# hedgepigdaniel/video-annotator

Hardware: AMD Instinct MI355X
Metric: stabilized frames/sec at 4K NV12, 1/2/4/8 GPU; remap % HBM roofline (higher is better)
Workload: dtype u8 pixels / f32 map / f64 rotations

## Files before the change

video-annotator_amd/csrc/vstab_warp_fused.hip:

```cpp
#include <algorithm>
#include <climits>
#include <cmath>
#include <cstdlib>

#include <hip/hip_ext.h>

#include "vstab_device.hpp"
#include "vstab_device10.hpp"
#include "vstab_internal.hpp"
#include "vstab_warp_args.hpp"
#include "vstab_warp_tile.hpp"

namespace vstab {

#ifdef VSTAB_DEV
#define VSTAB_STAMP(k)                                                                                                   \
    if (ta.timing && lane == 0) ta.timing[((size_t)blockIdx.x * 4 + (size_t)wave) * 8 + (k)] = __builtin_amdgcn_s_memrealtime()
#else
#define VSTAB_STAMP(k)
#endif

template <int RWB, int RW, int MODE, int FMT, bool CACHED, bool SPLIT, int DEPTH = 8, int BLEND = 0>
__device__ __forceinline__ bool warp_tile(const FusedArgs &ta, uint32_t *smem, const int x0, const int y0) {
    static_assert((DEPTH == 8 && FMT < 2) || (DEPTH == 10 && FMT >= 2), "10-bit pixels leave as 16-bit BGR (FMT 2) or P010 planes (FMT 3)");
    using SrcVec = typename std::conditional<DEPTH == 10, uint4, uint2>::type;
    constexpr uint32_t BPS = DEPTH == 10 ? 2 : 1;
    constexpr int TH = 4 * RW;
    constexpr int STAGE_MAX = StageTrips<RWB, RW>::value;
    constexpr int QB = CACHED ? 0 : QMAGIC_BITS;
    constexpr bool PIX8 = DEPTH == 10 && BLEND == VSTAB_BLEND_FP16;
    constexpr int PD = PIX8 ? 2 : 1;
    constexpr bool RS = map_mode_is_rs(MODE);
    constexpr int BASE = map_mode_base(MODE);
    uint32_t *const tile = smem + 8;
    const WarpArgs &a = ta.w;
    const int tid = threadIdx.x, lane = tid & 63, wave = __builtin_amdgcn_readfirstlane(tid >> 6);
    const float rfx = rcp_refined(a.p.ofx), rfy = rcp_refined(a.p.ofy);

    VSTAB_STAMP(0);
    if (wave == 0) {
        __builtin_amdgcn_s_setprio(3);
        probe_tile<TH, STAGE_MAX, MODE, CACHED>(ta, x0, y0, lane, rfx, rfy, smem);
        __builtin_amdgcn_s_setprio(VSTAB_WARP_PRIO);
    }
    __syncthreads();
    const int bx0 = __builtin_amdgcn_readfirstlane((int)smem[0]), by0 = __builtin_amdgcn_readfirstlane((int)smem[1]);
    const int wb = __builtin_amdgcn_readfirstlane((int)smem[2]), hb = __builtin_amdgcn_readfirstlane((int)smem[3]);
    const int box_state = __builtin_amdgcn_readfirstlane((int)smem[4]);
    if constexpr (SPLIT) {
        if (box_state == 2) return false;
    }
    const bool use_lds = box_state == 1;
    const int x = x0 + lane;
    VSTAB_STAMP(1);

    const int ux_n = wb >> 3, units = use_lds ? ux_n * (hb >> 1) : 0;
#ifdef VSTAB_DEV
    const int pw = (wb + ta.lds_pad) * PD;
#else
    const int pw = wb * PD;
#endif
    SrcVec y0w[STAGE_MAX], y1w[STAGE_MAX], uvw[STAGE_MAX];
    int ldsoff[STAGE_MAX];
    constexpr int ZERO_BLOCK = 1 << 24;
    if (use_lds) {
        const float rn = __builtin_amdgcn_rcpf((float)ux_n);
        int uy = (int)((float)tid * rn), ux = tid - uy * ux_n;
        if (ux < 0) ux += ux_n, uy--;
        if (ux >= ux_n) ux -= ux_n, uy++;
        int sy_ = (int)(256.0f * rn), sx_ = 256 - sy_ * ux_n;
        if (sx_ < 0) sx_ += ux_n, sy_--;
        if (sx_ >= ux_n) sx_ -= ux_n, sy_++;
        const uint32_t pitch_y = (uint32_t)a.pitch_y, pitch_uv = (uint32_t)a.pitch_uv;
#pragma unroll
        for (int it = 0; it < STAGE_MAX; it++) {
            if (it > 0 && units <= it * 256) {
                y0w[it] = y1w[it] = uvw[it] = SrcVec(), ldsoff[it] = -1;
                continue;
            }
            const bool valid = tid + it * 256 < units;
            const int gx = bx0 + 8 * ux, gy = by0 + 2 * uy;
            const bool inside = (uint32_t)gx < (uint32_t)(a.sw & ~7) && (uint32_t)gy < (uint32_t)a.sh;
            const uint32_t cx = (uint32_t)min(max(gx, 0), (a.sw & ~7) - 8), cy = (uint32_t)min(max(gy, 0), a.sh - 2);
            const uint32_t oy = __umul24(cy, pitch_y) + cx * BPS, ouv = __umul24(cy >> 1, pitch_uv) + cx * BPS;
            y0w[it] = *reinterpret_cast<const SrcVec *>(a.y + oy);
            y1w[it] = *reinterpret_cast<const SrcVec *>(a.y + (oy + pitch_y));
            uvw[it] = *reinterpret_cast<const SrcVec *>(a.uv + ouv);
            ldsoff[it] = valid ? (__mul24(2 * uy, pw) + 8 * PD * ux) | (inside ? 0 : ZERO_BLOCK) : -1;
            ux += sx_, uy += sy_;
            if (ux >= ux_n) ux -= ux_n, uy++;
        }
    } else {
#pragma unroll
        for (int it = 0; it < STAGE_MAX; it++) y0w[it] = y1w[it] = uvw[it] = SrcVec(), ldsoff[it] = -1;
    }

    VSTAB_STAMP(2);
    int qxb[RW], qyb[RW];
    {
        int unused_cx[RW / 2], unused_cy[RW / 2];
        const float unused_qm[4] = {QMAGIC, QMAGIC, QMAGIC, QMAGIC};
        map_phase<RW, MODE, CACHED, false>(ta, x, y0, wave, lane, rfx, rfy, qxb, qyb, unused_cx, unused_cy, unused_qm);
    }
#pragma unroll
    for (int j = 0; j < RW; j++) asm volatile("" : "+v"(qxb[j]), "+v"(qyb[j]) : : "memory");

    VSTAB_STAMP(3);
    if (use_lds) {
#pragma unroll
        for (int it = 0; it < STAGE_MAX; it++) {
            if (ldsoff[it] >= ZERO_BLOCK) {
                uint32_t *d = tile + (ldsoff[it] - ZERO_BLOCK);
                const uint4 z = make_uint4(0, 0, 0, 0);
#pragma unroll
                for (int q = 0; q < 2 * PD; q++) *reinterpret_cast<uint4 *>(d + 4 * q) = z, *reinterpret_cast<uint4 *>(d + pw + 4 * q) = z;
#ifdef VSTAB_DEV
            } else if (DEPTH == 8 && ldsoff[it] >= 0 && (ta.ablate & 4)) {
                uint32_t *d = tile + ldsoff[it];
                *reinterpret_cast<uint4 *>(d) = make_uint4(y0w[it].x, y0w[it].y, uvw[it].x, uvw[it].y);
                *reinterpret_cast<uint4 *>(d + 4) = make_uint4(y0w[it].y, y0w[it].x, uvw[it].x, uvw[it].y);
                *reinterpret_cast<uint4 *>(d + pw) = make_uint4(y1w[it].x, y1w[it].y, uvw[it].x, uvw[it].y);
                *reinterpret_cast<uint4 *>(d + pw + 4) = make_uint4(y1w[it].y, y1w[it].x, uvw[it].y, uvw[it].x);
#endif
            } else if (ldsoff[it] >= 0) {
                uint32_t *d = tile + ldsoff[it];
                if constexpr (DEPTH == 10) {
                    const uint32_t ya[4] = {y0w[it].x, y0w[it].y, y0w[it].z, y0w[it].w}, yb[4] = {y1w[it].x, y1w[it].y, y1w[it].z, y1w[it].w};
                    const uint32_t cw[4] = {uvw[it].x, uvw[it].y, uvw[it].z, uvw[it].w};
#pragma unroll
                    for (int half = 0; half < 2; half++) {
                        const ChromaTerm c0 = chroma_term10(cw[2 * half]), c1 = chroma_term10(cw[2 * half + 1]);
                        if constexpr (PIX8) {
                            const uint32_t la = ya[2 * half], lb = ya[2 * half + 1], ma = yb[2 * half], mb = yb[2 * half + 1];
                            const uint2 a0 = pack_bgr10h((int)((la & 0xffffu) >> 6), c0), a1 = pack_bgr10h((int)(la >> 22), c0);
                            const uint2 a2 = pack_bgr10h((int)((lb & 0xffffu) >> 6), c1), a3 = pack_bgr10h((int)(lb >> 22), c1);
                            const uint2 b0 = pack_bgr10h((int)((ma & 0xffffu) >> 6), c0), b1 = pack_bgr10h((int)(ma >> 22), c0);
                            const uint2 b2 = pack_bgr10h((int)((mb & 0xffffu) >> 6), c1), b3 = pack_bgr10h((int)(mb >> 22), c1);
                            *reinterpret_cast<uint4 *>(d + 8 * half) = make_uint4(a0.x, a0.y, a1.x, a1.y);
                            *reinterpret_cast<uint4 *>(d + 8 * half + 4) = make_uint4(a2.x, a2.y, a3.x, a3.y);
                            *reinterpret_cast<uint4 *>(d + pw + 8 * half) = make_uint4(b0.x, b0.y, b1.x, b1.y);
                            *reinterpret_cast<uint4 *>(d + pw + 8 * half + 4) = make_uint4(b2.x, b2.y, b3.x, b3.y);
                            continue;
                        }
                        uint4 r0, r1;
                        r0.x = pack_bgr10((int)((ya[2 * half] & 0xffffu) >> 6), c0), r0.y = pack_bgr10((int)(ya[2 * half] >> 22), c0);
                        r0.z = pack_bgr10((int)((ya[2 * half + 1] & 0xffffu) >> 6), c1), r0.w = pack_bgr10((int)(ya[2 * half + 1] >> 22), c1);
                        r1.x = pack_bgr10((int)((yb[2 * half] & 0xffffu) >> 6), c0), r1.y = pack_bgr10((int)(yb[2 * half] >> 22), c0);
                        r1.z = pack_bgr10((int)((yb[2 * half + 1] & 0xffffu) >> 6), c1), r1.w = pack_bgr10((int)(yb[2 * half + 1] >> 22), c1);
                        *reinterpret_cast<uint4 *>(d + 4 * half) = r0;
                        *reinterpret_cast<uint4 *>(d + pw + 4 * half) = r1;
                    }
                } else
#pragma unroll
                for (int half = 0; half < 2; half++) {
                    const uint32_t cw = half ? uvw[it].y : uvw[it].x, ya = half ? y0w[it].y : y0w[it].x, yb = half ? y1w[it].y : y1w[it].x;
                    const ChromaTerm c0 = chroma_term_folded(cw & 255, (cw >> 8) & 255);
                    const ChromaTerm c1 = chroma_term_folded((cw >> 16) & 255, cw >> 24);
                    uint4 r0, r1;
                    r0.x = pack_bgrx(ya & 255, c0), r0.y = pack_bgrx((ya >> 8) & 255, c0);
                    r0.z = pack_bgrx((ya >> 16) & 255, c1), r0.w = pack_bgrx(ya >> 24, c1);
                    r1.x = pack_bgrx(yb & 255, c0), r1.y = pack_bgrx((yb >> 8) & 255, c0);
                    r1.z = pack_bgrx((yb >> 16) & 255, c1), r1.w = pack_bgrx(yb >> 24, c1);
                    *reinterpret_cast<uint4 *>(d + 4 * half) = r0;
                    *reinterpret_cast<uint4 *>(d + pw + 4 * half) = r1;
                }
            }
        }
    }
    VSTAB_STAMP(4);
    __syncthreads();
    VSTAB_STAMP(5);

    const bool col_live = x < a.dw;
    uint32_t out[RW];
    {
        int cx = bx0 + (QB >> 5), cy = by0 + (QB >> 5);
        asm("" : "+s"(cx), "+s"(cy));
        const uint32_t wlim = use_lds ? (uint32_t)(wb - 1) : 0u, hlim = (uint32_t)(hb - 1);
        int Xr[RW], Yr[RW];
        const uint32_t wb4 = (uint32_t)pw << 2;
        uint32_t tile_lds = (uint32_t)(uintptr_t)(__attribute__((address_space(3))) uint32_t *)tile;
        asm("" : "+s"(tile_lds));
        uint32_t mxx = 0, mxy = 0;
#pragma unroll
        for (int j = 0; j < RW; j++) {
            Xr[j] = (qxb[j] >> 5) - cx, Yr[j] = (qyb[j] >> 5) - cy;
            mxx = max(mxx, (uint32_t)Xr[j]), mxy = max(mxy, (uint32_t)Yr[j]);
        }
        if (!__builtin_amdgcn_ballot_w64(mxx >= wlim || mxy >= hlim)) {
            constexpr int TG = RW < TAP_GROUP ? RW : TAP_GROUP;
            if constexpr (PIX8) {
#pragma unroll
                for (int j0 = 0; j0 < RW; j0 += TG) {
                    uint2 t0[TG], t1[TG], t2[TG], t3[TG];
#pragma unroll
                    for (int j = 0; j < TG; j++) {
                        uint32_t ax8, au;
                        asm("v_lshl_add_u32 %0, %1, 3, %2" : "=v"(ax8) : "v"(Xr[j0 + j]), "s"(tile_lds));
                        asm("v_mad_u32_u24 %0, %1, %2, %3" : "=v"(au) : "v"(Yr[j0 + j]), "s"(wb4), "v"(ax8));
                        const LdsPair *u = reinterpret_cast<const LdsPair *>(au), *l = reinterpret_cast<const LdsPair *>(au + wb4);
                        const u32x2 v0 = u[0], v1 = u[1], v2 = l[0], v3 = l[1];
                        t0[j] = make_uint2(v0.x, v0.y), t1[j] = make_uint2(v1.x, v1.y), t2[j] = make_uint2(v2.x, v2.y), t3[j] = make_uint2(v3.x, v3.y);
                    }
#pragma unroll
                    for (int j = 0; j < TG; j++) out[j0 + j] = blend_bgr10h(t0[j], t1[j], t2[j], t3[j], qxb[j0 + j] & 31, qyb[j0 + j] & 31);
                }
            } else
#pragma unroll
            for (int j0 = 0; j0 < RW; j0 += TG) {
                uint32_t t0[TG], t1[TG], t2[TG], t3[TG];
#pragma unroll
                for (int j = 0; j < TG; j++) {
                    uint32_t ax4, au;
                    asm("v_lshl_add_u32 %0, %1, 2, %2" : "=v"(ax4) : "v"(Xr[j0 + j]), "s"(tile_lds));
                    asm("v_mad_u32_u24 %0, %1, %2, %3" : "=v"(au) : "v"(Yr[j0 + j]), "s"(wb4), "v"(ax4));
                    const LdsWord *u = reinterpret_cast<const LdsWord *>(au), *l = reinterpret_cast<const LdsWord *>(au + wb4);
                    t0[j] = u[0], t1[j] = u[1], t2[j] = l[0], t3[j] = l[1];
                }
#pragma unroll
                for (int j = 0; j < TG; j++) {
#ifdef VSTAB_DEV
                    if (ta.ablate & 2) out[j0 + j] = t0[j] ^ t1[j] ^ t2[j] ^ t3[j] ^ (qxb[j0 + j] & 31) ^ (qyb[j0 + j] & 31);
                    else
#endif
                    out[j0 + j] = DEPTH == 10 ? blend_bgr10<BLEND>(t0[j], t1[j], t2[j], t3[j], qxb[j0 + j] & 31, qyb[j0 + j] & 31)
                                              : blend_bgrx(t0[j], t1[j], t2[j], t3[j], qxb[j0 + j] & 31, qyb[j0 + j] & 31);
                }
            }
        } else {
            uint32_t slow = 0;
#pragma unroll
            for (int j = 0; j < RW; j++) {
                const bool inbox = (uint32_t)Xr[j] < wlim && (uint32_t)Yr[j] < hlim;
                uint32_t v = 0;
                if (inbox) {
                    const uint32_t *t = tile + (__mul24(Yr[j], pw) + PD * Xr[j]);
                    if constexpr (PIX8)
                        v = blend_bgr10h(make_uint2(t[0], t[1]), make_uint2(t[2], t[3]), make_uint2(t[pw], t[pw + 1]), make_uint2(t[pw + 2], t[pw + 3]), qxb[j] & 31,
                                         qyb[j] & 31);
                    else
                        v = DEPTH == 10 ? blend_bgr10<BLEND>(t[0], t[1], t[pw], t[pw + 1], qxb[j] & 31, qyb[j] & 31)
                                        : blend_bgrx(t[0], t[1], t[pw], t[pw + 1], qxb[j] & 31, qyb[j] & 31);
                }
                out[j] = v;
                const bool live = col_live && y0 + wave * RW + j < a.dh;
                slow |= (!inbox && live ? 1u : 0u) << j;
            }
            if (__builtin_amdgcn_ballot_w64(slow != 0)) {
#pragma unroll 1
                for (int j = 0; j < RW; j++) {
                    int sx = qxb[0], sy = qyb[0];
#pragma unroll
                    for (int k = 1; k < RW; k++) sx = j == k ? qxb[k] : sx, sy = j == k ? qyb[k] : sy;
                    if ((slow >> j) & 1u) {
                        const uint32_t v = DEPTH == 10 ? gather_pixel10<BLEND>(a, sx - QB, sy - QB) : gather_pixel_far(a, sx - QB, sy - QB);
#pragma unroll
                        for (int k = 0; k < RW; k++) out[k] = j == k ? v : out[k];
                    }
                }
            }
        }
    }

    VSTAB_STAMP(6);
#ifdef VSTAB_DEV
    if (ta.ablate & 8) {
        uint32_t acc = 0;
#pragma unroll
        for (int j = 0; j < RW; j++) acc ^= out[j];
        if (acc == 0x12345678u) a.dst[0] = 1;
        return true;
    }
#endif
    const int ncols = min(64, a.dw - x0);
    if constexpr (FMT == 2) {
#pragma unroll
        for (int j = 0; j < RW; j++) {
            const int y = y0 + wave * RW + j;
            if (y >= a.dh) break;
            if (col_live) {
                uint16_t *o = reinterpret_cast<uint16_t *>(a.dst + ((size_t)(uint32_t)y * a.pitch_dst + (uint32_t)x * 6u));
                o[0] = (uint16_t)(out[j] & 1023u), o[1] = (uint16_t)((out[j] >> 10) & 1023u), o[2] = (uint16_t)(out[j] >> 20);
            }
        }
    } else if constexpr (FMT == 3) {
#pragma unroll
        for (int j = 0; j < RW; j++) {
            const int y = y0 + wave * RW + j;
            if (y >= a.dh) break;
            const int B = (int)(out[j] & 1023u), G = (int)((out[j] >> 10) & 1023u), R = (int)(out[j] >> 20);
            const uint32_t yb = (uint32_t)sat10((CRY * R + CGY * G + CBY * B + (1 << 19) + (64 << 20)) >> 20) << 6;
            const uint32_t y1 = (uint32_t)__builtin_amdgcn_mov_dpp((int)yb, 0x55, 0xf, 0xf, true);
            const uint32_t y2 = (uint32_t)__builtin_amdgcn_mov_dpp((int)yb, 0xaa, 0xf, 0xf, true);
            const uint32_t y3 = (uint32_t)__builtin_amdgcn_mov_dpp((int)yb, 0xff, 0xf, 0xf, true);
            uint16_t *o = reinterpret_cast<uint16_t *>(a.dst + (size_t)(uint32_t)y * a.pitch_dst) + x;
            if (!(lane & 3) && col_live) {
                if (ta.dst_vec_ok && x + 4 <= a.dw) {
                    *reinterpret_cast<uint2 *>(o) = make_uint2(yb | (y1 << 16), y2 | (y3 << 16));
                } else {
                    const uint32_t w[4] = {yb, y1, y2, y3};
                    for (int i = 0; i < 4 && x + i < a.dw; i++) o[i] = (uint16_t)w[i];
                }
            }
            if (!(y & 1)) {
                const uint32_t U = (uint32_t)sat10((CRU * R + CGU * G + CBU * B + (1 << 19) + (512 << 20)) >> 20) << 6;
                const uint32_t V = (uint32_t)sat10((CBU * R + CGV * G + CBV * B + (1 << 19) + (512 << 20)) >> 20) << 6;
                const uint32_t cb = U | (V << 16);
                const uint32_t c2 = (uint32_t)__builtin_amdgcn_mov_dpp((int)cb, 0xaa, 0xf, 0xf, true);
                uint16_t *c = reinterpret_cast<uint16_t *>(a.dst_uv + (size_t)(uint32_t)(y >> 1) * a.pitch_dst_uv) + x;
                if (!(lane & 3) && col_live) {
                    if (ta.dst_vec_ok && x + 2 < a.dw) {
                        *reinterpret_cast<uint2 *>(c) = make_uint2(cb, c2);
                    } else {
                        *reinterpret_cast<uint32_t *>(c) = cb;
                        if (x + 2 < a.dw) *reinterpret_cast<uint32_t *>(c + 2) = c2;
                    }
                }
            }
        }
    } else if constexpr (FMT == 0) {
        const int p0 = (4 * lane) / 3, m3 = lane - 3 * (lane / 3);
        const uint32_t sel = m3 == 0 ? 0x04020100u : m3 == 1 ? 0x05040201u : 0x06050402u;
        const int nbytes = 3 * ncols, nfull = nbytes >> 2, rem = nbytes & 3;
        if (ta.dst_vec_ok && ncols == 64 && y0 + wave * RW + RW <= a.dh) {
            uint32_t lo[RW], hi[RW];
#pragma unroll
            for (int j = 0; j < RW; j++) {
                lo[j] = (uint32_t)__builtin_amdgcn_ds_bpermute(4 * p0, (int)out[j]);
                hi[j] = (uint32_t)__builtin_amdgcn_ds_bpermute(4 * p0 + 4, (int)out[j]);
            }
            uint8_t *o = a.dst + ((size_t)(uint32_t)(y0 + wave * RW) * a.pitch_dst + (uint32_t)x0 * 3u);
            if (lane < 48) {
#pragma unroll
                for (int j = 0; j < RW; j++) {
                    *reinterpret_cast<uint32_t *>(o + (uint32_t)(4 * lane)) = __builtin_amdgcn_perm(hi[j], lo[j], sel);
                    o += a.pitch_dst;
                }
            }
        } else
#pragma unroll
// ... 204 lines not shown
```

video-annotator_amd/csrc/vstab_warp_planar.hip:

```cpp
#include <algorithm>
#include <climits>
#include <cmath>
#include <cstdlib>

#include <hip/hip_ext.h>

#include "vstab_device.hpp"
#include "vstab_device10.hpp"
#include "vstab_internal.hpp"
#include "vstab_warp_args.hpp"
#include "vstab_warp_tile.hpp"

namespace vstab {

typedef __attribute__((address_space(3))) uint8_t LdsU8;
typedef __attribute__((address_space(3))) uint16_t LdsU16;
typedef __attribute__((address_space(3))) uint32_t LdsU32;
typedef unsigned short u16x2 __attribute__((ext_vector_type(2)));

template <int DEPTH>
struct Planar {
    static constexpr int BPS = DEPTH == 10 ? 2 : 1;
    static constexpr int BW = 16 / BPS;
    static constexpr int BLACK_Y = DEPTH == 10 ? 64 : 16;
// ... 147 lines not shown
        }
    }
    int qxb[RW], qyb[RW], qcx[RW / 2], qcy[RW / 2];
    {
        const float qm[4] = {QMAGIC - (float)(32 * bx0), QMAGIC - (float)(32 * by0), QMAGIC - (float)(32 * (bx0 >> 1)), QMAGIC - (float)(32 * (by0 >> 1))};
        map_phase<RW, MODE, false, true, true>(ta, x, y0, wave, lane, rfx, rfy, qxb, qyb, qcx, qcy, qm);
    }
#pragma unroll
    for (int j = 0; j < RW; j++) asm volatile("" : "+v"(qxb[j]), "+v"(qyb[j]) : : "memory");
#pragma unroll
    for (int j = 0; j < RW / 2; j++) asm volatile("" : "+v"(qcx[j]), "+v"(qcy[j]));

    __syncthreads();

    const bool col_live = x < a.dw;
    constexpr int OSH = DEPTH == 10 ? 0 : 16;
    int out[RW];
    uint32_t outw[(RW + 1) / 2];
    {
        int mnx = qxb[0], mxx = qxb[0], mny = qyb[0], mxy = qyb[0];
#pragma unroll
        for (int j = 1; j < RW; j++) mnx = min(mnx, qxb[j]), mxx = max(mxx, qxb[j]), mny = min(mny, qyb[j]), mxy = max(mxy, qyb[j]);
        const int hix = QB + 32 * (wb - 1), hiy = QB + 32 * (hb - 1);
        const bool outside_box = !use_lds || mnx < QB || mxx >= hix || mny < QB || mxy >= hiy;
#ifdef VSTAB_DEV
        if (ta.ablate & 2) {
#pragma unroll
            for (int j = 0; j < RW; j++) out[j] = qxb[j] ^ qyb[j], outw[j / 2] = (uint32_t)(qxb[j] ^ qyb[j]);
        } else
#endif
        if (!__builtin_amdgcn_ballot_w64(outside_box)) {
            constexpr int TG = RW < 4 ? RW : 4;
#pragma unroll
            for (int j0 = 0; j0 < RW; j0 += TG) {
                uint32_t t0[TG], t1[TG];
#pragma unroll
                for (int j = 0; j < TG; j++) {
                    const uint32_t xr = __builtin_amdgcn_ubfe((uint32_t)qxb[j0 + j], 5, 17), yr = __builtin_amdgcn_ubfe((uint32_t)qyb[j0 + j], 5, 17);
                    uint32_t ad;
                    if constexpr (DEPTH == 10) {
                        asm("v_mad_u32_u24 %0, %1, %2, %3" : "=v"(ad) : "v"(yr), "s"(pw), "v"(xr << 1));
                        const volatile LdsU16 *u = reinterpret_cast<const volatile LdsU16 *>((__attribute__((address_space(3))) uint8_t *)tile + ad);
                        const volatile LdsU16 *l = reinterpret_cast<const volatile LdsU16 *>((__attribute__((address_space(3))) uint8_t *)tile + (ad + (uint32_t)pw));
                        t0[j] = (uint32_t)u[0] | ((uint32_t)u[1] << 16), t1[j] = (uint32_t)l[0] | ((uint32_t)l[1] << 16);
                    } else {
                        asm("v_mad_u32_u24 %0, %1, %2, %3" : "=v"(ad) : "v"(yr), "s"(pw), "v"(xr));
                        const LdsU8 *u = (__attribute__((address_space(3))) uint8_t *)tile + ad, *l = (__attribute__((address_space(3))) uint8_t *)tile + (ad + (uint32_t)pw);
                        t0[j] = (uint32_t)u[0] | ((uint32_t)u[1] << 16), t1[j] = (uint32_t)l[0] | ((uint32_t)l[1] << 16);
                    }
                }
                if constexpr (DEPTH == 10) {
#pragma unroll
                    for (int j = 0; j < TG; j += 2) {
                        const uint32_t qa = (uint32_t)qxb[j0 + j], qb = (uint32_t)qxb[j0 + j + 1], ra = (uint32_t)qyb[j0 + j], rb = (uint32_t)qyb[j0 + j + 1];
                        uint32_t v2;
                        if constexpr (BLEND == VSTAB_BLEND_FP16) {
                            const uint32_t p00 = sig10_x2(__builtin_amdgcn_perm(t0[j + 1], t0[j], 0x05040100u)), p01 = sig10_x2(__builtin_amdgcn_perm(t0[j + 1], t0[j], 0x07060302u));
                            const uint32_t p10 = sig10_x2(__builtin_amdgcn_perm(t1[j + 1], t1[j], 0x05040100u)), p11 = sig10_x2(__builtin_amdgcn_perm(t1[j + 1], t1[j], 0x07060302u));
                            const uint32_t fx2 = __builtin_amdgcn_perm(qb, qa, 0x05040100u) & 0x001f001fu, fy2 = __builtin_amdgcn_perm(rb, ra, 0x05040100u) & 0x001f001fu;
                            v2 = blend10h_x2(half_of10_x2(p00), half_of10_x2(p01), half_of10_x2(p10), half_of10_x2(p11), frac_half_x2(fx2), frac_half_x2(fy2));
                        } else {
                            uint32_t v[2];
#pragma unroll
                            for (int k = 0; k < 2; k++) {
                                const uint32_t fx = (k ? qb : qa) & 31u, fy = (k ? rb : ra) & 31u;
                                const uint32_t wx = fx * 65535u + 32u;
                                const uint32_t h0 = __builtin_amdgcn_udot2(__builtin_bit_cast(u16x2, sig10_x2(t0[j + k])), __builtin_bit_cast(u16x2, wx), 0u, false);
                                const uint32_t h1 = __builtin_amdgcn_udot2(__builtin_bit_cast(u16x2, sig10_x2(t1[j + k])), __builtin_bit_cast(u16x2, wx), 0u, false);
                                v[k] = (uint32_t)lerp_rows(h0, h1, fy);
                            }
                            v2 = v[0] | (v[1] << 16);
                        }
                        outw[(j0 + j) / 2] = v2 << 6;
                    }
                } else {
#pragma unroll
                    for (int j = 0; j < TG; j++) {
                        const uint32_t fx = (uint32_t)qxb[j0 + j] & 31u, fy = (uint32_t)qyb[j0 + j] & 31u;
                        out[j0 + j] = (int)blend8_scaled(t0[j], t1[j], fx * 262140u + 128u, fy);
                    }
                }
            }
        } else {
#pragma unroll 1
            for (int j = 0; j < RW; j++) {
                int sx = qxb[0], sy = qyb[0];
#pragma unroll
                for (int k = 1; k < RW; k++) sx = j == k ? qxb[k] : sx, sy = j == k ? qyb[k] : sy;
                const int v = gather_sample<DEPTH, BLEND>(a.y, a.pitch_y, a.sw, a.sh, 1, 0, sx - QB + 32 * bx0, sy - QB + 32 * by0, P::BLACK_Y) << OSH;
#pragma unroll
                for (int k = 0; k < RW; k++) out[k] = j == k ? v : out[k];
            }
            if constexpr (DEPTH == 10) {
#pragma unroll
                for (int k = 0; k < RW; k += 2) outw[k / 2] = ((uint32_t)out[k] | ((uint32_t)out[k + 1] << 16)) << 6;
            }
        }
    }

    int cu[NS], cv[NS];
    uint32_t cw[NS];
    {
        int ccx[NS], ccy[NS];
        const bool odd = lane & 1;
#pragma unroll
        for (int s = 0; s < NS; s++) {
            const int so = 2 * s + 1 < CR ? 2 * s + 1 : 2 * s;
            const int ox = __builtin_amdgcn_mov_dpp(qcx[so], 0xa0, 0xf, 0xf, true), oy = __builtin_amdgcn_mov_dpp(qcy[so], 0xa0, 0xf, 0xf, true);
            ccx[s] = odd ? ox : qcx[2 * s], ccy[s] = odd ? oy : qcy[2 * s];
        }
        int mnx = ccx[0], mxx = ccx[0], mny = ccy[0], mxy = ccy[0];
#pragma unroll
        for (int s = 1; s < NS; s++) mnx = min(mnx, ccx[s]), mxx = max(mxx, ccx[s]), mny = min(mny, ccy[s]), mxy = max(mxy, ccy[s]);
        const int cbx0 = bx0 >> 1, cby0 = by0 >> 1, cwb = wb >> 1, chb = hb >> 1;
        const int hix = QB + 32 * (cwb - 1), hiy = QB + 32 * (chb - 1);
        const bool outside_box = !use_lds || mnx < QB || mxx >= hix || mny < QB || mxy >= hiy;
#ifdef VSTAB_DEV
        if (ta.ablate & 4) {
#pragma unroll
            for (int s = 0; s < NS; s++) cu[s] = ccx[s], cv[s] = ccy[s], cw[s] = (uint32_t)(ccx[s] ^ ccy[s]);
        } else
#endif
        if (!__builtin_amdgcn_ballot_w64(outside_box)) {
            constexpr uint32_t CPX = 2 * BPS;
            const __attribute__((address_space(3))) uint8_t *const ctile = (__attribute__((address_space(3))) uint8_t *)tile + luma_bytes;
#pragma unroll
            for (int s = 0; s < NS; s++) {
                const uint32_t xr = __builtin_amdgcn_ubfe((uint32_t)ccx[s], 5, 17), yr = __builtin_amdgcn_ubfe((uint32_t)ccy[s], 5, 17);
                const uint32_t fx = (uint32_t)ccx[s] & 31u, fy = (uint32_t)ccy[s] & 31u;
                uint32_t ad;
                asm("v_mad_u32_u24 %0, %1, %2, %3" : "=v"(ad) : "v"(yr), "s"(pw), "v"(xr * CPX));
                if constexpr (DEPTH == 10) {
                    const LdsU32 *pt = reinterpret_cast<const LdsU32 *>(ctile + ad), *pb = reinterpret_cast<const LdsU32 *>(ctile + (ad + (uint32_t)pw));
                    const uint32_t a0 = sig10_x2(pt[0]), a1 = sig10_x2(pt[1]), b0 = sig10_x2(pb[0]), b1 = sig10_x2(pb[1]);
                    uint32_t v2;
                    if constexpr (BLEND == VSTAB_BLEND_FP16) {
                        v2 = blend10h_x2(half_of10_x2(a0), half_of10_x2(a1), half_of10_x2(b0), half_of10_x2(b1), frac_half_x2(fx * 0x10001u), frac_half_x2(fy * 0x10001u));
                    } else {
                        const u16x2 wx = __builtin_bit_cast(u16x2, fx * 65535u + 32u);
                        auto row = [&](uint32_t l, uint32_t r, uint32_t sel) { return __builtin_amdgcn_udot2(__builtin_bit_cast(u16x2, __builtin_amdgcn_perm(r, l, sel)), wx, 0u, false); };
                        const uint32_t u = (uint32_t)lerp_rows(row(a0, a1, 0x05040100u), row(b0, b1, 0x05040100u), fy);
                        const uint32_t v = (uint32_t)lerp_rows(row(a0, a1, 0x07060302u), row(b0, b1, 0x07060302u), fy);
                        v2 = u | (v << 16);
                    }
                    cw[s] = v2 << 6;
                } else {
                    const LdsU16 *pt = reinterpret_cast<const LdsU16 *>(ctile + ad), *pb = reinterpret_cast<const LdsU16 *>(ctile + (ad + (uint32_t)pw));
                    const uint32_t tt = (uint32_t)pt[0] | ((uint32_t)pt[1] << 16), tb = (uint32_t)pb[0] | ((uint32_t)pb[1] << 16);
                    const uint32_t wu = fx * 262140u + 128u;
                    cu[s] = (int)blend8_scaled(tt, tb, wu, fy), cv[s] = (int)blend8_scaled(tt, tb, wu << 8, fy);
                }
            }
        } else {
#pragma unroll 1
            for (int s = 0; s < NS; s++) {
                int sx = ccx[0], sy = ccy[0];
#pragma unroll
                for (int k = 1; k < NS; k++) sx = s == k ? ccx[k] : sx, sy = s == k ? ccy[k] : sy;
                const int u = gather_sample<DEPTH, BLEND>(a.uv, a.pitch_uv, a.sw >> 1, a.sh >> 1, 2, 0, sx - QB + 32 * cbx0, sy - QB + 32 * cby0, P::BLACK_C) << OSH;
                const int v = gather_sample<DEPTH, BLEND>(a.uv, a.pitch_uv, a.sw >> 1, a.sh >> 1, 2, 1, sx - QB + 32 * cbx0, sy - QB + 32 * cby0, P::BLACK_C) << OSH;
#pragma unroll
                for (int k = 0; k < NS; k++) cu[k] = s == k ? u : cu[k], cv[k] = s == k ? v : cv[k];
            }
            if constexpr (DEPTH == 10) {
#pragma unroll
                for (int k = 0; k < NS; k++) cw[k] = ((uint32_t)cu[k] | ((uint32_t)cv[k] << 16)) << 6;
            }
        }
    }

#ifdef VSTAB_DEV
    if (ta.ablate & 8) {
        int acc = 0;
#pragma unroll
        for (int j = 0; j < RW; j++) acc ^= DEPTH == 10 ? (int)outw[j / 2] : out[j];
#pragma unroll
        for (int s = 0; s < NS; s++) acc ^= DEPTH == 10 ? (int)cw[s] : cu[s] ^ cv[s];
        if (acc == 0x12345678) a.dst[0] = 1;
        return true;
    }
#endif
    const int yw = y0 + wave * RW;
    const int ncols = min(64, a.dw - x0);
    if (ta.dst_vec_ok && ncols == 64 && yw + RW <= a.dh) {
        uint8_t *const scr = scratch + wave * P::SCRATCH_PER_WAVE;
        uint8_t *const scr_c = scr + RW * 64 * BPS;
        {
            uint8_t *w = scr + lane * BPS;
#pragma unroll
            for (int j = 0; j < RW; j++) {
                if constexpr (DEPTH == 10) *reinterpret_cast<u16_alias *>(w + j * 128) = (uint16_t)(j & 1 ? outw[j / 2] >> 16 : outw[j / 2]);
                else w[j * 64] = (uint8_t)((uint32_t)out[j] >> 16);
            }
            uint8_t *wc = scr_c + (lane & 1) * 64 * BPS + (lane >> 1) * 2 * BPS;
            if (CR > 1 || !(lane & 1)) {
#pragma unroll
                for (int s = 0; s < NS; s++) {
                    if constexpr (DEPTH == 10) *reinterpret_cast<u32_alias *>(wc + s * 256) = cw[s];
                    else *reinterpret_cast<u16_alias *>(wc + s * 128) = (uint16_t)__builtin_amdgcn_perm((uint32_t)cv[s], (uint32_t)cu[s], 0x0c0c0602u);
                }
            }
        }
        constexpr int NBY = RW * BPS, NBC = RW * BPS / 2;
        constexpr int LPR_Y = 64 * BPS / NBY, LPR_C = 64 * BPS / NBC;
        {
            const int r = lane / LPR_Y, c = (lane % LPR_Y) * NBY;
            scratch_to_global<NBY>(scr + lane * NBY, a.dst + ((size_t)(uint32_t)(yw + r) * a.pitch_dst + (uint32_t)x0 * BPS + (uint32_t)c));
        }
        {
            const int r = lane / LPR_C, c = (lane % LPR_C) * NBC;
            scratch_to_global<NBC>(scr_c + lane * NBC, a.dst_uv + ((size_t)(uint32_t)((yw >> 1) + r) * a.pitch_dst_uv + (uint32_t)x0 * BPS + (uint32_t)c));
        }
    } else {
#pragma unroll
        for (int j = 0; j < RW; j++) {
            const int y = yw + j;
            if (col_live && y < a.dh) {
                uint8_t *o = a.dst + ((size_t)(uint32_t)y * a.pitch_dst + (uint32_t)x * BPS);
                if constexpr (DEPTH == 10) {
                    const uint32_t wd = j & 1 ? outw[j / 2] >> 16 : outw[j / 2];
                    o[0] = (uint8_t)(wd & 255u), o[1] = (uint8_t)(wd >> 8);
                } else o[0] = (uint8_t)((uint32_t)out[j] >> 16);
            }
        }
        const int xc = x0 + (lane & ~1);
#pragma unroll
        for (int s = 0; s < NS; s++) {
            const int y = yw + 2 * ((lane & 1) + 2 * s);
            if (xc < a.dw && y < a.dh && (lane & 1) + 2 * s < CR) {
                uint8_t *o = a.dst_uv + ((size_t)(uint32_t)(y >> 1) * a.pitch_dst_uv + (uint32_t)xc * BPS);
                if constexpr (DEPTH == 10) o[0] = (uint8_t)cw[s], o[1] = (uint8_t)(cw[s] >> 8), o[2] = (uint8_t)(cw[s] >> 16), o[3] = (uint8_t)(cw[s] >> 24);
                else o[0] = (uint8_t)((uint32_t)cu[s] >> 16), o[1] = (uint8_t)((uint32_t)cv[s] >> 16);
            }
        }
    }
    return true;
// ... 98 lines not shown
```

video-annotator_amd/csrc/vstab_warp_tile.hpp:

```cpp
#pragma once
#include <algorithm>
#include <climits>
#include <cmath>
#include <cstdlib>

#include "vstab_device.hpp"
#include "vstab_internal.hpp"
#include "vstab_warp_args.hpp"

namespace vstab {

#ifndef VSTAB_WARP_WAVES
#define VSTAB_WARP_WAVES 7
#endif
#ifndef VSTAB_WARP_PRIO
#define VSTAB_WARP_PRIO 1
#endif
#ifndef VSTAB_MAP_GROUP
#define VSTAB_MAP_GROUP 2
#endif
#ifndef VSTAB_TAP_GROUP
#define VSTAB_TAP_GROUP 4
#endif
constexpr int MAP_GROUP = VSTAB_MAP_GROUP;
constexpr int TAP_GROUP = VSTAB_TAP_GROUP;
constexpr float QMAGIC = 12582912.0f;
constexpr int QMAGIC_BITS = 0x4B400000;

typedef short short2v __attribute__((ext_vector_type(2)));
typedef __attribute__((address_space(3))) uint32_t LdsWord;
typedef uint32_t u32x2 __attribute__((ext_vector_type(2)));
typedef __attribute__((address_space(3))) u32x2 LdsPair;

__device__ __forceinline__ uint32_t pk_min_i16(uint32_t a, uint32_t b) {
    return __builtin_bit_cast(uint32_t, __builtin_elementwise_min(__builtin_bit_cast(short2v, a), __builtin_bit_cast(short2v, b)));
}
__device__ __forceinline__ uint32_t pk_max_i16(uint32_t a, uint32_t b) {
    return __builtin_bit_cast(uint32_t, __builtin_elementwise_max(__builtin_bit_cast(short2v, a), __builtin_bit_cast(short2v, b)));
}

template <bool MAX>
__device__ __forceinline__ uint32_t wave_reduce_pk_i16(uint32_t v) {
    constexpr uint32_t ident = MAX ? 0x80008000u : 0x7fff7fffu;
#define VSTAB_STEP(ctrl, rmask)                                                                              \
    {                                                                                                        \
        const uint32_t t = (uint32_t)__builtin_amdgcn_update_dpp((int)ident, (int)v, ctrl, rmask, 0xf, false); \
        v = MAX ? pk_max_i16(v, t) : pk_min_i16(v, t);                                                       \
    }
    VSTAB_STEP(0x111, 0xf) VSTAB_STEP(0x112, 0xf) VSTAB_STEP(0x114, 0xf) VSTAB_STEP(0x118, 0xf)
    VSTAB_STEP(0x142, 0xa) VSTAB_STEP(0x143, 0xc)
#undef VSTAB_STEP
    return (uint32_t)__builtin_amdgcn_readlane((int)v, 63);
}

__device__ __forceinline__ uint32_t gather_pixel_far(const WarpArgs &a, int sx, int sy) {
    const int X = sx >> 5, Y = sy >> 5;
    if (!(X < a.sw && X + 1 >= 0 && Y < a.sh && Y + 1 >= 0)) return 0;
    return gather_pixel(a, sx, sy);
}

template <int RWB, int RW>
struct StageTrips {
    static constexpr int value = RW == 8 ? 3 : RW == 4 ? 2 : (RWB == 8 ? 2 : 1);
};

template <int TH, int STAGE_MAX, int MODE, bool CACHED, bool PLANAR = false, int BLOCK_W = 8>
__device__ __forceinline__ void probe_tile(const FusedArgs &ta, int x0, int y0, int lane, float rfx, float rfy, uint32_t *hdr) {
    constexpr bool RS = map_mode_is_rs(MODE);
    constexpr int BASE = map_mode_base(MODE);
    const WarpArgs &a = ta.w;
    int px, py;
    const int l16 = lane & 15, side = (l16 * (TH - 1) + 7) / 15;
    if (lane < 16) px = 4 * l16, py = 0;
    else if (lane < 32) px = 4 * l16 + 3, py = TH - 1;
    else if (lane < 48) px = 0, py = side;
    else px = 63, py = side;
    px = min(px, a.dw - 1 - x0), py = min(py, a.dh - 1 - y0);
    int qx, qy;
    if constexpr (CACHED) {
        const int2 q = ta.qmap[(size_t)(y0 + py) * ta.qpitch + (x0 + px)];
        qx = q.x, qy = q.y;
    } else {
        float ax, ay;
        if constexpr (BASE == MAP_CREATEMAP_CL || BASE == MAP_FISH_TO_RECT || BASE == MAP_CREATEMAP_CL_OPENCL) {
            const float vx = ((float)(x0 + px) - a.p.ocx) * rfx, vy = ((float)(y0 + py) - a.p.ocy) * rfy;
            float m[9];
#pragma unroll
            for (int k = 0; k < 9; k++) m[k] = a.p.r[k];
            if constexpr (RS) {
                const float t = (float)(y0 + py) * __builtin_amdgcn_rcpf(ta.rs_den);
#pragma unroll
                for (int k = 0; k < 9; k++) m[k] = __builtin_fmaf(t, ta.rs_d[k], a.p.r[k]);
            }
            const float wx = __builtin_fmaf(m[0], vx, __builtin_fmaf(m[1], vy, m[2]));
            const float wy = __builtin_fmaf(m[3], vx, __builtin_fmaf(m[4], vy, m[5]));
            const float wz = __builtin_fmaf(m[6], vx, __builtin_fmaf(m[7], vy, m[8]));
            const float rz = __builtin_amdgcn_rcpf(wz), ux = wx * rz, uy = wy * rz;
            const float q = __builtin_fmaf(ux, ux, uy * uy), rs = __builtin_amdgcn_rsqf(q), rad = q * rs;
            const bool inv = rad > 1.0f;
            const float t = inv ? rs : rad, s2 = t * t;
            float g = 0.0028423243202269077f;
            g = __builtin_fmaf(g, s2, -0.016053270548582077f);
            g = __builtin_fmaf(g, s2, 0.04269874095916748f);
            g = __builtin_fmaf(g, s2, -0.07508683204650879f);
            g = __builtin_fmaf(g, s2, 0.1064559817314148f);
            g = __builtin_fmaf(g, s2, -0.14205896854400635f);
            g = __builtin_fmaf(g, s2, 0.19993145763874054f);
            g = __builtin_fmaf(g, s2, -0.33333125710487366f);
            float at = __builtin_fmaf(t * s2, g, t);
            at = inv ? 1.57079637050628662109375f - at : at;
            const float k = at * rs;
            ax = __builtin_fmaf(ux * k, ta.p32.ifx32, ta.p32.icx32), ay = __builtin_fmaf(uy * k, ta.p32.ify32, ta.p32.icy32);
            if (BASE == MAP_FISH_TO_RECT && !(wz > 0.0f)) ax = ay = __builtin_nanf("");
        } else {
            const float vx = div_with_rcp((float)(x0 + px) - a.p.ocx, a.p.ofx, rfx);
            const float vy = div_with_rcp((float)(y0 + py) - a.p.ocy, a.p.ofy, rfy);
            const ColTerm ct = {a.p.r[0] * vx, a.p.r[3] * vx, a.p.r[6] * vx};
            const RowTerm rt = {a.p.r[1] * vy, a.p.r[4] * vy, a.p.r[7] * vy};
            map_pixel_ex<BASE>(ta.p32, a.p, ct, rt, vx, vy, ax, ay);
        }
        qx = __float_as_int(ax + QMAGIC) - QMAGIC_BITS, qy = __float_as_int(ay + QMAGIC) - QMAGIC_BITS;
    }
    int Xc, Yc;
    asm("v_med3_i32 %0, %1, -1, %2" : "=v"(Xc) : "v"(qx >> 5), "s"(a.sw));
    asm("v_med3_i32 %0, %1, -1, %2" : "=v"(Yc) : "v"(qy >> 5), "s"(a.sh));
    const uint32_t pk = ((uint32_t)Xc & 0xffffu) | ((uint32_t)Yc << 16);
    const uint32_t mn = wave_reduce_pk_i16<false>(pk), mx = wave_reduce_pk_i16<true>(pk);
    const int mnx = (int)(short)(mn & 0xffffu), mny = (int)mn >> 16, mxx = (int)(short)(mx & 0xffffu), mxy = (int)mx >> 16;
    constexpr int LO_M = PLANAR ? 2 : 1, HI_M = PLANAR ? 5 : 2, CAP = PLANAR ? 1 : 0, BM = BLOCK_W - 1;
    const int lox = max(mnx - LO_M, -LO_M), hix = min(mxx + HI_M, a.sw + CAP), loy = max(mny - LO_M, -LO_M), hiy = min(mxy + HI_M, a.sh + CAP);
    const int bx0 = lox & ~BM, by0 = loy & ~1;
    const int wb = (hix + 1 - bx0 + BM) & ~BM, hb = (hiy + 1 - by0 + 1) & ~1;
    const bool have = mnx < a.sw && mxx >= -1 && mny < a.sh && mxy >= -1;
    const bool stageable = have && a.sw >= BLOCK_W && ta.src_vec_ok && ((a.sw & BM) == 0 || bx0 + wb <= (a.sw & ~BM));
#ifdef VSTAB_DEV
    const bool fits = (wb + ta.lds_pad) * hb <= ta.lds_capacity_px && (wb >> 3) * (hb >> 1) <= STAGE_MAX * 256;
#else
    const bool fits = wb * hb <= ta.lds_capacity_px && (wb / BLOCK_W) * (hb >> 1) <= STAGE_MAX * 256 && (!PLANAR || wb / BLOCK_W <= 64);
#endif
    if (lane == 0) {
        *reinterpret_cast<uint4 *>(hdr) = make_uint4((uint32_t)bx0, (uint32_t)by0, (uint32_t)wb, (uint32_t)hb);
        hdr[4] = stageable ? (fits ? 1u : 2u) : 0u;
    }
}

#define VSTAB_EACH _Pragma("unroll") for (int c = 0; c < NP; c++)
template <int NP, bool FISH_TO_RECT>
__device__ __forceinline__ void map_pairs_ieee(float icx32, float icy32, float ifx32, float ify32, const f32x2 (&wx)[NP], const f32x2 (&wy)[NP],
                                               const f32x2 (&wz)[NP], f32x2 (&ax)[NP], f32x2 (&ay)[NP]) {
    f32x2 rz[NP], e[NP], px[NP], py[NP], ex[NP], ey[NP], q[NP], y[NP], g[NP], h[NP], d[NP], rad[NP], rr[NP], t[NP], s[NP], at[NP], k[NP];
    i32x2 inv[NP];
    const f32x2 one = splat2(1.0f), half = splat2(0.5f);
    VSTAB_EACH rz[c] = (f32x2){__builtin_amdgcn_rcpf(wz[c].x), __builtin_amdgcn_rcpf(wz[c].y)};
    VSTAB_EACH e[c] = fma2(-wz[c], rz[c], one);
    VSTAB_EACH rz[c] = fma2(e[c], rz[c], rz[c]);
    VSTAB_EACH px[c] = wx[c] * rz[c], py[c] = wy[c] * rz[c];
    VSTAB_EACH ex[c] = fma2(-wz[c], px[c], wx[c]), ey[c] = fma2(-wz[c], py[c], wy[c]);
    VSTAB_EACH px[c] = fma2(ex[c], rz[c], px[c]), py[c] = fma2(ey[c], rz[c], py[c]);
    VSTAB_EACH ex[c] = fma2(-wz[c], px[c], wx[c]), ey[c] = fma2(-wz[c], py[c], wy[c]);
    VSTAB_EACH px[c] = fma2(ex[c], rz[c], px[c]), py[c] = fma2(ey[c], rz[c], py[c]);
    VSTAB_EACH q[c] = px[c] * px[c] + py[c] * py[c];
    VSTAB_EACH y[c] = (f32x2){__builtin_amdgcn_rsqf(q[c].x), __builtin_amdgcn_rsqf(q[c].y)};
    VSTAB_EACH g[c] = q[c] * y[c], h[c] = half * y[c];
    VSTAB_EACH e[c] = fma2(-h[c], g[c], half);
    VSTAB_EACH h[c] = fma2(h[c], e[c], h[c]), g[c] = fma2(g[c], e[c], g[c]);
    VSTAB_EACH d[c] = fma2(-g[c], g[c], q[c]);
    VSTAB_EACH rad[c] = fma2(d[c], h[c], g[c]);
    VSTAB_EACH rr[c] = (f32x2){__builtin_amdgcn_rcpf(rad[c].x), __builtin_amdgcn_rcpf(rad[c].y)};
    VSTAB_EACH e[c] = fma2(-rad[c], rr[c], one);
    VSTAB_EACH rr[c] = fma2(e[c], rr[c], rr[c]);
    VSTAB_EACH inv[c] = rad[c] > one, t[c] = one * rr[c];
    VSTAB_EACH e[c] = fma2(-rad[c], t[c], one);
    VSTAB_EACH t[c] = fma2(e[c], rr[c], t[c]);
    VSTAB_EACH e[c] = fma2(-rad[c], t[c], one);
    VSTAB_EACH t[c] = fma2(e[c], rr[c], t[c]);
    VSTAB_EACH t[c] = inv[c] ? t[c] : rad[c];
    VSTAB_EACH s[c] = t[c] * t[c];
    VSTAB_EACH g[c] = fma2(splat2(0.0028423243202269077f), s[c], splat2(-0.016053270548582077f));
    VSTAB_EACH g[c] = fma2(g[c], s[c], splat2(0.04269874095916748f));
    VSTAB_EACH g[c] = fma2(g[c], s[c], splat2(-0.07508683204650879f));
    VSTAB_EACH g[c] = fma2(g[c], s[c], splat2(0.1064559817314148f));
    VSTAB_EACH g[c] = fma2(g[c], s[c], splat2(-0.14205896854400635f));
    VSTAB_EACH g[c] = fma2(g[c], s[c], splat2(0.19993145763874054f));
    VSTAB_EACH g[c] = fma2(g[c], s[c], splat2(-0.33333125710487366f));
    VSTAB_EACH at[c] = fma2(t[c] * s[c], g[c], t[c]);
    VSTAB_EACH at[c] = inv[c] ? (splat2(1.57079637050628662109375f) - at[c]) + splat2(-4.37113900018624283e-8f) : at[c];
    VSTAB_EACH k[c] = at[c] * rr[c];
    VSTAB_EACH e[c] = fma2(-rad[c], k[c], at[c]);
    VSTAB_EACH k[c] = fma2(e[c], rr[c], k[c]);
    VSTAB_EACH e[c] = fma2(-rad[c], k[c], at[c]);
    VSTAB_EACH k[c] = fma2(e[c], rr[c], k[c]);
    if constexpr (FISH_TO_RECT) {
        VSTAB_EACH k[c] = (q[c] == splat2(0.0f)) ? one : k[c];
    }
    VSTAB_EACH ax[c] = splat2(icx32) + (px[c] * k[c]) * splat2(ifx32), ay[c] = splat2(icy32) + (py[c] * k[c]) * splat2(ify32);
    if constexpr (FISH_TO_RECT) {
        VSTAB_EACH {
            const i32x2 ok = wz[c] > splat2(0.0f);
            ax[c] = ok ? ax[c] : splat2(__builtin_nanf("")), ay[c] = ok ? ay[c] : splat2(__builtin_nanf(""));
        }
    }
}

__device__ __forceinline__ bool map_q_irregular(uint32_t qmin, uint32_t qmax) { return qmin < 0x17800000u  || qmax > 0x67800000u ; }
template <int NP>
__device__ __forceinline__ void map_pairs_ocl(float icx32, float icy32, float ifx32, float ify32, const f32x2 (&wx)[NP], const f32x2 (&wy)[NP],
                                              const f32x2 (&wz)[NP], f32x2 (&ax)[NP], f32x2 (&ay)[NP], uint32_t &qmin, uint32_t &qmax) {
    f32x2 rz[NP], px[NP], py[NP], q[NP], rad[NP], rr[NP], t[NP], s[NP], p[NP], r[NP], k[NP];
    i32x2 inv[NP];
    VSTAB_EACH rz[c] = (f32x2){__builtin_amdgcn_rcpf(wz[c].x), __builtin_amdgcn_rcpf(wz[c].y)};
    VSTAB_EACH px[c] = wx[c] * rz[c], py[c] = wy[c] * rz[c];
    VSTAB_EACH q[c] = fma2(py[c], py[c], px[c] * px[c]);
    VSTAB_EACH rad[c] = (f32x2){__builtin_amdgcn_sqrtf(q[c].x), __builtin_amdgcn_sqrtf(q[c].y)};
    VSTAB_EACH {
        qmin = min(min(qmin, __float_as_uint(q[c].x)), __float_as_uint(q[c].y));
        qmax = max(max(qmax, __float_as_uint(q[c].x)), __float_as_uint(q[c].y));
    }
    VSTAB_EACH rr[c] = (f32x2){__builtin_amdgcn_rcpf(rad[c].x), __builtin_amdgcn_rcpf(rad[c].y)};
    VSTAB_EACH inv[c] = rad[c] > splat2(1.0f), t[c] = inv[c] ? rr[c] : rad[c];
    VSTAB_EACH s[c] = t[c] * t[c];
    VSTAB_EACH p[c] = fma2(splat2(f32_bits(0x3b2d2a58u)), s[c], splat2(f32_bits(0xbc7a590cu)));
    VSTAB_EACH p[c] = fma2(s[c], p[c], splat2(f32_bits(0x3d29fb3fu)));
    VSTAB_EACH p[c] = fma2(s[c], p[c], splat2(f32_bits(0xbd97d4d7u)));
    VSTAB_EACH p[c] = fma2(s[c], p[c], splat2(f32_bits(0x3dd931b2u)));
    VSTAB_EACH p[c] = fma2(s[c], p[c], splat2(f32_bits(0xbe1160e6u)));
// ... 177 lines not shown
```

Before: 27780.

## Skip map and gather work for tiles proven to map outside the source

The probe wave now tries to prove, from the tile's border samples and their neighbour deltas, that the whole output tile maps outside the source image for computed fisheye maps. When it can, the fused kernel skips the per-pixel map computation and the gather and writes black. In the slow path, and in the planar kernel, a wave-wide check also emits black directly when no pixel lands inside the source. This removes wasted map math and far gathers on border regions, at the cost of extra reductions in the probe and a heuristic bound (slack from neighbour deltas) whose correctness depends on the map being smooth.

```diff
diff --git a/video-annotator_amd/csrc/vstab_warp_fused.hip b/video-annotator_amd/csrc/vstab_warp_fused.hip
--- a/video-annotator_amd/csrc/vstab_warp_fused.hip
+++ b/video-annotator_amd/csrc/vstab_warp_fused.hip
@@ -15,9 +15,12 @@
 
 #ifdef VSTAB_DEV
 #define VSTAB_STAMP(k)                                                                                                   \
-    if (ta.timing && lane == 0) ta.timing[((size_t)blockIdx.x * 4 + (size_t)wave) * 8 + (k)] = __builtin_amdgcn_s_memrealtime()
+    if (ta.timing && lane == 0) ta.timing[((size_t)blockIdx.x * 4 + (size_t)wave) * 9 + (k)] = __builtin_amdgcn_s_memrealtime()
+#define VSTAB_NOTE(v)                                                                                                    \
+    if (ta.timing && lane == 0) ta.timing[((size_t)blockIdx.x * 4 + (size_t)wave) * 9 + 8] = (unsigned long long)(v)
 #else
 #define VSTAB_STAMP(k)
+#define VSTAB_NOTE(v)
 #endif
 
 template <int RWB, int RW, int MODE, int FMT, bool CACHED, bool SPLIT, int DEPTH = 8, int BLEND = 0>
@@ -40,7 +43,7 @@
     VSTAB_STAMP(0);
     if (wave == 0) {
         __builtin_amdgcn_s_setprio(3);
-        probe_tile<TH, STAGE_MAX, MODE, CACHED>(ta, x0, y0, lane, rfx, rfy, smem);
+        probe_tile<TH, STAGE_MAX, MODE, CACHED, false, 8, probe_proves_outside<MODE, CACHED>()>(ta, x0, y0, lane, rfx, rfy, smem);
         __builtin_amdgcn_s_setprio(VSTAB_WARP_PRIO);
     }
     __syncthreads();
@@ -51,8 +54,10 @@
         if (box_state == 2) return false;
     }
     const bool use_lds = box_state == 1;
+    const bool tile_outside = probe_proves_outside<MODE, CACHED>() && box_state == 3;
     const int x = x0 + lane;
     VSTAB_STAMP(1);
+    VSTAB_NOTE(1 + box_state);
 
     const int ux_n = wb >> 3, units = use_lds ? ux_n * (hb >> 1) : 0;
 #ifdef VSTAB_DEV
@@ -97,7 +102,10 @@
 
     VSTAB_STAMP(2);
     int qxb[RW], qyb[RW];
-    {
+    if (tile_outside) {
+#pragma unroll
+        for (int j = 0; j < RW; j++) qxb[j] = qyb[j] = 0;
+    } else {
         int unused_cx[RW / 2], unused_cy[RW / 2];
         const float unused_qm[4] = {QMAGIC, QMAGIC, QMAGIC, QMAGIC};
         map_phase<RW, MODE, CACHED, false>(ta, x, y0, wave, lane, rfx, rfy, qxb, qyb, unused_cx, unused_cy, unused_qm);
@@ -167,6 +175,21 @@
             }
         }
     }
+    int Xr[RW], Yr[RW];
+    uint32_t mxx = 0, mxy = 0;
+    if (tile_outside) {
+#pragma unroll
+        for (int j = 0; j < RW; j++) Xr[j] = Yr[j] = 0;
+    } else {
+        int cx = bx0 + (QB >> 5), cy = by0 + (QB >> 5);
+        asm("" : "+s"(cx), "+s"(cy));
+#pragma unroll
+        for (int j = 0; j < RW; j++) {
+            Xr[j] = (qxb[j] >> 5) - cx, Yr[j] = (qyb[j] >> 5) - cy;
+            mxx = max(mxx, (uint32_t)Xr[j]), mxy = max(mxy, (uint32_t)Yr[j]);
+        }
+        asm volatile("" : "+v"(mxx), "+v"(mxy));
+    }
     VSTAB_STAMP(4);
     __syncthreads();
     VSTAB_STAMP(5);
@@ -174,20 +197,14 @@
     const bool col_live = x < a.dw;
     uint32_t out[RW];
     {
-        int cx = bx0 + (QB >> 5), cy = by0 + (QB >> 5);
-        asm("" : "+s"(cx), "+s"(cy));
         const uint32_t wlim = use_lds ? (uint32_t)(wb - 1) : 0u, hlim = (uint32_t)(hb - 1);
-        int Xr[RW], Yr[RW];
         const uint32_t wb4 = (uint32_t)pw << 2;
         uint32_t tile_lds = (uint32_t)(uintptr_t)(__attribute__((address_space(3))) uint32_t *)tile;
         asm("" : "+s"(tile_lds));
-        uint32_t mxx = 0, mxy = 0;
-#pragma unroll
-        for (int j = 0; j < RW; j++) {
-            Xr[j] = (qxb[j] >> 5) - cx, Yr[j] = (qyb[j] >> 5) - cy;
-            mxx = max(mxx, (uint32_t)Xr[j]), mxy = max(mxy, (uint32_t)Yr[j]);
-        }
-        if (!__builtin_amdgcn_ballot_w64(mxx >= wlim || mxy >= hlim)) {
+        if (tile_outside) {
+#pragma unroll
+            for (int j = 0; j < RW; j++) out[j] = 0;
+        } else if (!__builtin_amdgcn_ballot_w64(mxx >= wlim || mxy >= hlim)) {
             constexpr int TG = RW < TAP_GROUP ? RW : TAP_GROUP;
             if constexpr (PIX8) {
 #pragma unroll
@@ -228,34 +245,47 @@
                 }
             }
         } else {
-            uint32_t slow = 0;
+            uint32_t inside = 0;
 #pragma unroll
             for (int j = 0; j < RW; j++) {
-                const bool inbox = (uint32_t)Xr[j] < wlim && (uint32_t)Yr[j] < hlim;
-                uint32_t v = 0;
-                if (inbox) {
-                    const uint32_t *t = tile + (__mul24(Yr[j], pw) + PD * Xr[j]);
-                    if constexpr (PIX8)
-                        v = blend_bgr10h(make_uint2(t[0], t[1]), make_uint2(t[2], t[3]), make_uint2(t[pw], t[pw + 1]), make_uint2(t[pw + 2], t[pw + 3]), qxb[j] & 31,
-                                         qyb[j] & 31);
-                    else
-                        v = DEPTH == 10 ? blend_bgr10<BLEND>(t[0], t[1], t[pw], t[pw + 1], qxb[j] & 31, qyb[j] & 31)
-                                        : blend_bgrx(t[0], t[1], t[pw], t[pw + 1], qxb[j] & 31, qyb[j] & 31);
-                }
-                out[j] = v;
+                const int X = (qxb[j] - QB) >> 5, Y = (qyb[j] - QB) >> 5;
                 const bool live = col_live && y0 + wave * RW + j < a.dh;
-                slow |= (!inbox && live ? 1u : 0u) << j;
-            }
-            if (__builtin_amdgcn_ballot_w64(slow != 0)) {
+                inside |= (live && X < a.sw && X + 1 >= 0 && Y < a.sh && Y + 1 >= 0 ? 1u : 0u) << j;
+            }
+            if (!__builtin_amdgcn_ballot_w64(inside != 0)) {
+                VSTAB_NOTE(1 + box_state + 16);
+#pragma unroll
+                for (int j = 0; j < RW; j++) out[j] = 0;
+            } else {
+                VSTAB_NOTE(1 + box_state + 32);
+                uint32_t slow = 0;
+#pragma unroll
+                for (int j = 0; j < RW; j++) {
+                    const bool inbox = (uint32_t)Xr[j] < wlim && (uint32_t)Yr[j] < hlim;
+                    uint32_t v = 0;
+                    if (inbox) {
+                        const uint32_t *t = tile + (__mul24(Yr[j], pw) + PD * Xr[j]);
+                        if constexpr (PIX8)
+                            v = blend_bgr10h(make_uint2(t[0], t[1]), make_uint2(t[2], t[3]), make_uint2(t[pw], t[pw + 1]), make_uint2(t[pw + 2], t[pw + 3]), qxb[j] & 31,
+                                             qyb[j] & 31);
+                        else
+                            v = DEPTH == 10 ? blend_bgr10<BLEND>(t[0], t[1], t[pw], t[pw + 1], qxb[j] & 31, qyb[j] & 31)
+                                            : blend_bgrx(t[0], t[1], t[pw], t[pw + 1], qxb[j] & 31, qyb[j] & 31);
+                    }
+                    out[j] = v;
+                    slow |= (!inbox ? inside & (1u << j) : 0u);
+                }
+                if (__builtin_amdgcn_ballot_w64(slow != 0)) {
 #pragma unroll 1
-                for (int j = 0; j < RW; j++) {
-                    int sx = qxb[0], sy = qyb[0];
-#pragma unroll
-                    for (int k = 1; k < RW; k++) sx = j == k ? qxb[k] : sx, sy = j == k ? qyb[k] : sy;
-                    if ((slow >> j) & 1u) {
-                        const uint32_t v = DEPTH == 10 ? gather_pixel10<BLEND>(a, sx - QB, sy - QB) : gather_pixel_far(a, sx - QB, sy - QB);
-#pragma unroll
-                        for (int k = 0; k < RW; k++) out[k] = j == k ? v : out[k];
+                    for (int j = 0; j < RW; j++) {
+                        int sx = qxb[0], sy = qyb[0];
+#pragma unroll
+                        for (int k = 1; k < RW; k++) sx = j == k ? qxb[k] : sx, sy = j == k ? qyb[k] : sy;
+                        if ((slow >> j) & 1u) {
+                            const uint32_t v = DEPTH == 10 ? gather_pixel10<BLEND>(a, sx - QB, sy - QB) : gather_pixel_far(a, sx - QB, sy - QB);
+#pragma unroll
+                            for (int k = 0; k < RW; k++) out[k] = j == k ? v : out[k];
+                        }
                     }
                 }
             }
diff --git a/video-annotator_amd/csrc/vstab_warp_planar.hip b/video-annotator_amd/csrc/vstab_warp_planar.hip
--- a/video-annotator_amd/csrc/vstab_warp_planar.hip
+++ b/video-annotator_amd/csrc/vstab_warp_planar.hip
@@ -253,6 +253,16 @@
                 }
             }
         } else {
+            bool in_src = false;
+#pragma unroll
+            for (int j = 0; j < RW; j++) {
+                const int X = ((qxb[j] - QB) >> 5) + bx0, Y = ((qyb[j] - QB) >> 5) + by0;
+                in_src |= !(X >= a.sw || X + 1 < 0 || Y >= a.sh || Y + 1 < 0);
+            }
+            if (!__builtin_amdgcn_ballot_w64(in_src)) {
+#pragma unroll
+                for (int j = 0; j < RW; j++) out[j] = P::BLACK_Y << OSH;
+            } else
 #pragma unroll 1
             for (int j = 0; j < RW; j++) {
                 int sx = qxb[0], sy = qyb[0];
@@ -323,6 +333,16 @@
                 }
             }
         } else {
+            bool in_src = false;
+#pragma unroll
+            for (int s = 0; s < NS; s++) {
+                const int X = ((ccx[s] - QB) >> 5) + cbx0, Y = ((ccy[s] - QB) >> 5) + cby0;
+                in_src |= !(X >= (a.sw >> 1) || X + 1 < 0 || Y >= (a.sh >> 1) || Y + 1 < 0);
+            }
+            if (!__builtin_amdgcn_ballot_w64(in_src)) {
+#pragma unroll
+                for (int s = 0; s < NS; s++) cu[s] = cv[s] = P::BLACK_C << OSH;
+            } else
 #pragma unroll 1
             for (int s = 0; s < NS; s++) {
                 int sx = ccx[0], sy = ccy[0];
diff --git a/video-annotator_amd/csrc/vstab_warp_tile.hpp b/video-annotator_amd/csrc/vstab_warp_tile.hpp
--- a/video-annotator_amd/csrc/vstab_warp_tile.hpp
+++ b/video-annotator_amd/csrc/vstab_warp_tile.hpp
@@ -64,7 +64,14 @@
     static constexpr int value = RW == 8 ? 3 : RW == 4 ? 2 : (RWB == 8 ? 2 : 1);
 };
 
-template <int TH, int STAGE_MAX, int MODE, bool CACHED, bool PLANAR = false, int BLOCK_W = 8>
+constexpr int OUTSIDE_SLACK = 2;
+constexpr float OUTSIDE_WZ_MIN = 1e-4f;
+template <int MODE, bool CACHED>
+constexpr bool probe_proves_outside() {
+    return !CACHED && !map_mode_is_rs(MODE) &&
+           (map_mode_base(MODE) == MAP_CREATEMAP_CL || map_mode_base(MODE) == MAP_FISH_TO_RECT || map_mode_base(MODE) == MAP_CREATEMAP_CL_OPENCL);
+}
+template <int TH, int STAGE_MAX, int MODE, bool CACHED, bool PLANAR = false, int BLOCK_W = 8, bool PROVE_OUTSIDE = false>
 __device__ __forceinline__ void probe_tile(const FusedArgs &ta, int x0, int y0, int lane, float rfx, float rfy, uint32_t *hdr) {
     constexpr bool RS = map_mode_is_rs(MODE);
     constexpr int BASE = map_mode_base(MODE);
@@ -77,6 +84,7 @@
     else px = 63, py = side;
     px = min(px, a.dw - 1 - x0), py = min(py, a.dh - 1 - y0);
     int qx, qy;
+    bool sane = false;
     if constexpr (CACHED) {
         const int2 q = ta.qmap[(size_t)(y0 + py) * ta.qpitch + (x0 + px)];
         qx = q.x, qy = q.y;
@@ -112,6 +120,7 @@
             const float k = at * rs;
             ax = __builtin_fmaf(ux * k, ta.p32.ifx32, ta.p32.icx32), ay = __builtin_fmaf(uy * k, ta.p32.ify32, ta.p32.icy32);
             if (BASE == MAP_FISH_TO_RECT && !(wz > 0.0f)) ax = ay = __builtin_nanf("");
+            if constexpr (PROVE_OUTSIDE) sane = wz > OUTSIDE_WZ_MIN && __builtin_fabsf(ax) < 4194304.0f && __builtin_fabsf(ay) < 4194304.0f;
         } else {
             const float vx = div_with_rcp((float)(x0 + px) - a.p.ocx, a.p.ofx, rfx);
             const float vy = div_with_rcp((float)(y0 + py) - a.p.ocy, a.p.ofy, rfy);
@@ -138,9 +147,26 @@
 #else
     const bool fits = wb * hb <= ta.lds_capacity_px && (wb / BLOCK_W) * (hb >> 1) <= STAGE_MAX * 256 && (!PLANAR || wb / BLOCK_W <= 64);
 #endif
+    bool outside = false;
+    if constexpr (PROVE_OUTSIDE) {
+        static_assert(probe_proves_outside<MODE, CACHED>() && !PLANAR, "the rule is argued for the computed fisheye maps of the fused kernel only");
+        if (mnx == a.sw || mxx == -1 || mny == a.sh || mxy == -1) {
+            const int X = qx >> 5, Y = qy >> 5;
+            const int Xn = __builtin_amdgcn_update_dpp(X, X, 0x111, 0xf, 0xf, false), Yn = __builtin_amdgcn_update_dpp(Y, Y, 0x111, 0xf, 0xf, false);
+            const int Xs = min(max(X, -32767), 32767), Ys = min(max(Y, -32767), 32767);
+            const int dX = min(abs(X - Xn), 32767), dY = min(abs(Y - Yn), 32767);
+            const uint32_t ex = wave_reduce_pk_i16<true>(((uint32_t)(-Xs) & 0xffffu) | ((uint32_t)Xs << 16));
+            const uint32_t ey = wave_reduce_pk_i16<true>(((uint32_t)(-Ys) & 0xffffu) | ((uint32_t)Ys << 16));
+            const uint32_t ed = wave_reduce_pk_i16<true>((uint32_t)dX | ((uint32_t)dY << 16));
+            const int minX = -(int)(short)(ex & 0xffffu), maxX = (int)ex >> 16, minY = -(int)(short)(ey & 0xffffu), maxY = (int)ey >> 16;
+            const int Mx = (int)(ed & 0xffffu) + OUTSIDE_SLACK, My = (int)(ed >> 16) + OUTSIDE_SLACK;
+            const bool all_sane = __builtin_amdgcn_ballot_w64(sane) == ~0ull;
+            outside = all_sane && (minX - Mx >= a.sw || maxX + Mx < -1 || minY - My >= a.sh || maxY + My < -1);
+        }
+    }
     if (lane == 0) {
         *reinterpret_cast<uint4 *>(hdr) = make_uint4((uint32_t)bx0, (uint32_t)by0, (uint32_t)wb, (uint32_t)hb);
-        hdr[4] = stageable ? (fits ? 1u : 2u) : 0u;
+        hdr[4] = outside ? 3u : stageable ? (fits ? 1u : 2u) : 0u;
     }
 }
 
```

After: 29130, median of 6. 4.9% higher.
